# thomasfork/aircraft_trajectory_optimization

Hardware: AMD Instinct MI355X
Metric: SQP iters/sec (batched) + lap-time err vs CasADi, 50×4 collocation (higher is better)
Workload: dtype f64; 1 GPU; racetrack_parametric_esp_drone_colloc_N50_K4_cold_start_batched_sqp; N=50, K=4, nz=13, nu=4, batch_per_gpu=512, global_batch=512, max_iter=47, layout=interleaved, parallelism=instances sharded x1

## Files before the change

### aircraft_trajectory_optimization_amd/csrc/ato_capi.hip

```cpp
#include <hip/hip_runtime.h>
#include <string>
#include <exception>
#include <new>
#include <cstdlib>
#include <cstring>
#include <algorithm>
#include "ato_kernels.hpp"

#include "ato_handle.hpp"

static thread_local std::string g_last_error;

static int fail(int code, const std::string& msg) {
    g_last_error = msg;
    return code;
}

void ato_internal_set_error(const std::string& msg) { g_last_error = msg; }

#define ATO_HIP(call)                                                                        \
    do {                                                                                     \
        hipError_t e_ = (call);                                                              \
        if (e_ != hipSuccess) return fail(ATO_ERR_HIP, std::string(#call) + ": " + hipGetErrorString(e_)); \
    } while (0)
// ... 254 lines not shown
        (void)hipFree(h->d_dJ);
        h->d_dJ = nullptr;
        return fail(ATO_ERR_HIP, "hessian scratch: out of device memory");
    }
    h->hess_reserved = max_batch;
    h->hess_colors = g;
    return ATO_OK;
}

int ato_reserve(ato_handle* h, int32_t max_batch) {
    if (!h || max_batch < 1) return fail(ATO_ERR_ARG, "bad reserve arguments");
    if (h->hess_ready) {
        int rc = hess_reserve(h, max_batch);
        if (rc) return rc;
    }
    if (max_batch <= h->reserved) return ATO_OK;
    if (h->d_fpart) {
        ATO_HIP(hipDeviceSynchronize());
        ATO_HIP(hipFree(h->d_fpart));
    }
    h->d_fpart = nullptr;
    h->reserved = 0;
    ATO_HIP(hipMalloc(&h->d_fpart, (size_t)h->L.p.N * max_batch * sizeof(double)));
    h->reserved = max_batch;
    return ATO_OK;
}

}

template <class T>
static int eval_impl(ato_handle* h, int32_t batch, int32_t layout, const T* w, T* g, T* jac, T* f,
                     T* grad_f, void* stream) {
    if (!h) return fail(ATO_ERR_ARG, "null handle");
    if (batch < 1) return fail(ATO_ERR_ARG, "batch must be >= 1");
    if (layout != ATO_LAYOUT_INTERLEAVED && layout != ATO_LAYOUT_INSTANCE_MAJOR)
        return fail(ATO_ERR_ARG, "unknown layout");
    if (!w) return fail(ATO_ERR_ARG, "w is null");
    const bool wf = f || grad_f;
    if (wf && !(f && grad_f)) return fail(ATO_ERR_ARG, "f and grad_f must be requested together");
    if (wf && batch > h->reserved) {
        int rc = ato_reserve(h, batch);
        if (rc) return rc;
    }
    const bool tiled = batch > h->lf_max_batch && h->eval_tile > 0;
    const ato::ProbD& p = batch <= h->lf_max_batch || (tiled && h->tile_lf) ? h->pd_lf : h->pd;
    hipError_t e = hipSuccess;
    ato::with_model(p, [&]<class M>() {
        hipEvent_t* ev = nullptr;
        const bool sample = h->timing_stride <= 1 || h->timing_seen % h->timing_stride == 0;
        if (!h->events.empty()) ++h->timing_seen;
        if (sample && (size_t)(h->timed_calls + 1) * 3 <= h->events.size())
            ev = &h->events[(size_t)h->timed_calls++ * 3];
        e = ato::launch_eval<M, T>(p, batch, layout, w, g, jac, grad_f, f, (T*)h->d_fpart, (hipStream_t)stream,
                                   ev, tiled ? h->eval_tile : 0);
    });
    if (e != hipSuccess) return fail(ATO_ERR_HIP, std::string("kernel launch: ") + hipGetErrorString(e));
// ... 342 lines not shown
```

### aircraft_trajectory_optimization_amd/csrc/ato_ipm.hip

```cpp
#include <hip/hip_runtime.h>
#include <cmath>
#include <string>
#include "../../include/ato_ipm.h"
#include "../../include/ato.h"

void ato_internal_set_error(const std::string& msg);

namespace {

constexpr int CH = 32;
constexpr int CB = 64;
constexpr int QMAX = 9;

__device__ __forceinline__ double nmax(double a, double b) {
    return (a != a || b != b) ? __builtin_nan("") : (a > b ? a : b);
}
__device__ __forceinline__ double nmin(double a, double b) {
    return (a != a || b != b) ? __builtin_nan("") : (a < b ? a : b);
}
__device__ __forceinline__ bool fin(double v) { return fabs(v) < INFINITY; }

struct Parts {
    int len[4];
    int c0[5];
// ... 1174 lines not shown
    const int k0 = blockIdx.y * RROWS, k1 = min(n0 + m, k0 + RROWS);
    for (int k = k0 + (threadIdx.x >> 6); k < k1; k += 4) {
        const long long o = (long long)k * W + b;
        if (k < n0) {
            x[o] = xb[o];
        } else {
            const long long d = (long long)(k - n0) * W + b;
            const double y = xb[o], rp = x[o], rn = x[o + (long long)m * W];
            x[o] = (rp + y) / dp[d];
            x[o + (long long)m * W] = (rn - y) / dn[d];
            x[o + 2LL * m * W] = y;
        }
    }
}

}

extern "C" {

int ato_ipm_perturb(int32_t op, int32_t W, int32_t m, const double* prm, int64_t* hdeg, int64_t* jdeg,
                    int64_t* diters, int64_t* test, double* dx, double* dc, double* dx_last, double* dc_last,
                    const double* mu, uint8_t* pend, const int32_t* inertia, double* dw_out, double* dc_out,
                    uint8_t* tosolve, const uint8_t* fin, void* stream) {
    if (op < 0 || op > 2 || W < 0 || !prm) return fail(ATO_ERR_ARG, "ato_ipm_perturb: arguments");
    if (W == 0) return 0;
    if (!hdeg || !jdeg || !diters || !test || !dx || !dc || !dx_last || !dc_last || !mu || !pend ||
        (op == 1 && (!inertia || !dw_out || !dc_out || !tosolve)) || (op == 2 && (!tosolve || !fin)))
        return fail(ATO_ERR_ARG, "ato_ipm_perturb: arguments");
    const PertPrm o{prm[0], prm[1], prm[2], prm[3], prm[4], prm[5], prm[6], prm[7], (long long)prm[8]};
    hipLaunchKernelGGL(k_perturb, dim3((W + CB - 1) / CB), dim3(CB), 0, static_cast<hipStream_t>(stream), (int)op, W,
// ... 307 lines not shown
                       static_cast<hipStream_t>(stream), n0, m, W, x, dp, dn, xb);
    return check_launch("ato_ipm_resto_kkt_rhs");
}

int ato_ipm_resto_kkt_expand(int32_t n0, int32_t m, int32_t W, const double* xb, const double* dp, const double* dn,
                             const uint8_t* mask, double* x, void* stream) {
    if (n0 < 0 || m < 0 || W < 0 || ((n0 + m) && W && (!x || !xb || !mask || (m && (!dp || !dn)))))
        return fail(ATO_ERR_ARG, "ato_ipm_resto_kkt_expand: arguments");
    if (n0 + m == 0 || W == 0) return 0;
    if ((n0 + m + RROWS - 1) / RROWS > GRID_Y_MAX) return fail(ATO_ERR_ARG, "ato_ipm_resto_kkt_expand: too many rows");
    hipLaunchKernelGGL(k_resto_kkt_expand, dim3((W + 63) / 64, (n0 + m + RROWS - 1) / RROWS), dim3(256), 0,
                       static_cast<hipStream_t>(stream), n0, m, W, xb, dp, dn, mask, x);
    return check_launch("ato_ipm_resto_kkt_expand");
}

}
```

### aircraft_trajectory_optimization_amd/native.py

```python
import ctypes
import os
from typing import Optional, Tuple

import numpy as np

KMAX = 9
GEOM_WIDTH = 16

ATO_MODEL_DRONE, ATO_MODEL_POINT = 0, 1
ATO_ATT_ESP, ATO_ATT_YPR, ATO_ATT_DCM = 0, 1, 2
ATO_FRAME_GLOBAL, ATO_FRAME_PARAMETRIC = 0, 1
ATO_TRANS_COLLOCATION, ATO_TRANS_RK4 = 0, 1
ATO_GATE_CIRCLE, ATO_GATE_SQUARE = 0, 1
ATO_LAYOUT_INTERLEAVED, ATO_LAYOUT_INSTANCE_MAJOR = 0, 1
ATO_AUDIT_NCH = 14
ATO_GATECHECK_NCH = 9
GATE_MAX = 64
ATO_OK, ATO_ERR_ARG, ATO_ERR_UNSUPPORTED, ATO_ERR_HIP, ATO_ERR_STATE = 0, -1, -2, -3, -4
ABI_VERSION = 3
CPC_MAX = 16

_c_double_p = ctypes.POINTER(ctypes.c_double)


# ... 98 lines not shown

class AtoIpmDims(ctypes.Structure):
    _fields_ = [('n', ctypes.c_int32), ('m', ctypes.c_int32), ('mi', ctypes.c_int32), ('meq', ctypes.c_int32),
                ('iin', ctypes.c_void_p), ('ieq', ctypes.c_void_p), ('W', ctypes.c_int32)]


class AtoIpmBounds(ctypes.Structure):
    _fields_ = [('xL', ctypes.c_void_p), ('xU', ctypes.c_void_p), ('dL', ctypes.c_void_p), ('dU', ctypes.c_void_p)]


IPM_SYMBOLS = ('ato_ipm_work_size', 'ato_ipm_errors', 'ato_ipm_rhs', 'ato_ipm_direction', 'ato_ipm_measures',
               'ato_ipm_multipliers', 'ato_ipm_filter_accept', 'ato_ipm_kkt_diag', 'ato_ipm_perturb',
               'ato_ipm_status', 'ato_ipm_barrier', 'ato_ipm_filter_multi', 'ato_ipm_refine_work',
               'ato_ipm_refine_pass', 'ato_ipm_refine_decide', 'ato_ipm_resto_rows', 'ato_ipm_js_jty',
               'ato_ipm_kmul_residual', 'ato_ipm_resto_eval', 'ato_ipm_resto_hess', 'ato_ipm_resto_kkt_pack',
               'ato_ipm_resto_kkt_diag', 'ato_ipm_resto_kkt_rhs', 'ato_ipm_resto_kkt_expand')

EXPORTED_SYMBOLS = ('ato_create', 'ato_destroy', 'ato_sizes', 'ato_sparsity', 'ato_bounds',
                    'ato_reserve', 'ato_eval', 'ato_eval_f32', 'ato_hess_sparsity', 'ato_hess_eval',
                    'ato_mesh_create', 'ato_mesh_destroy', 'ato_mesh_signed_distance',
                    'ato_timing', 'ato_timing_read', 'ato_timing_stride', 'ato_last_error', 'ato_version',
                    'ato_kkt_create', 'ato_kkt_destroy', 'ato_kkt_reserve', 'ato_kkt_factor', 'ato_kkt_solve',
                    'ato_kkt_residual', 'ato_kkt_residual_list', 'ato_set_instance_spheres',
                    'ato_sphere_rows', 'ato_gradf_mode', 'ato_gradf_sparsity', 'ato_replay_set_lift',
                    'ato_replay', 'ato_remesh', 'ato_mesh_signed_distance_strided', 'ato_clearance_set_line',
                    'ato_clearance', 'ato_audit', 'ato_gatecheck', 'ato_gatecheck_set_gates',
                    'ato_gatecheck_launches') + IPM_SYMBOLS


def library_path() -> str:
    return os.environ.get('ATO_LIB_PATH') or os.path.join(os.path.dirname(os.path.abspath(__file__)), '_lib',
                                                          'libato.so')


def declare(lib: ctypes.CDLL, prefix: str = 'ato') -> ctypes.CDLL:
    vp = ctypes.c_void_p
    i32p = ctypes.POINTER(ctypes.c_int32)
    getattr(lib, f'{prefix}_last_error').restype = ctypes.c_char_p
    if prefix == 'ato':
        lib.ato_version.restype = ctypes.c_char_p
        lib.ato_create.argtypes = [ctypes.POINTER(AtoProblemDesc), ctypes.POINTER(vp)]
        lib.ato_destroy.argtypes = [vp]
        lib.ato_sizes.argtypes = [vp, i32p, i32p, i32p]
        lib.ato_sparsity.argtypes = [vp, ctypes.POINTER(i32p), ctypes.POINTER(i32p)]
        lib.ato_bounds.argtypes = [vp, _c_double_p, _c_double_p]
        lib.ato_reserve.argtypes = [vp, ctypes.c_int32]
        lib.ato_eval.argtypes = [vp, ctypes.c_int32, ctypes.c_int32, vp, vp, vp, vp, vp, vp]
        lib.ato_eval_f32.argtypes = [vp, ctypes.c_int32, ctypes.c_int32, vp, vp, vp, vp, vp, vp]
        lib.ato_hess_sparsity.argtypes = [vp, i32p, ctypes.POINTER(i32p), ctypes.POINTER(i32p), i32p]
        lib.ato_hess_eval.argtypes = [vp, ctypes.c_int32, ctypes.c_int32, vp, vp, vp, vp, vp]
        lib.ato_mesh_create.argtypes = [vp, ctypes.c_int32, vp, ctypes.c_int32, ctypes.POINTER(vp)]
        lib.ato_mesh_destroy.argtypes = [vp]
        lib.ato_mesh_signed_distance.argtypes = [vp, ctypes.c_int32, vp, vp, vp, vp]
        lib.ato_timing.argtypes = [vp, ctypes.c_int32]
        lib.ato_timing_read.argtypes = [vp, _c_double_p, _c_double_p, i32p]
        lib.ato_timing_stride.argtypes = [vp, ctypes.c_int32]
        lib.ato_set_instance_spheres.argtypes = [vp, vp, ctypes.c_int64]
        lib.ato_sphere_rows.argtypes = [vp, i32p]
        lib.ato_gradf_mode.argtypes = [vp, ctypes.c_int32]
        lib.ato_gradf_sparsity.argtypes = [vp, i32p, i32p]
        lib.ato_replay_set_lift.argtypes = [vp, vp]
# ... 34 lines not shown
        lib.ato_ipm_perturb.argtypes = [ctypes.c_int32] * 3 + [vp] * 16 + [vp]
        lib.ato_ipm_status.argtypes = [ctypes.c_int32] + [vp] * 11 + [vp]
        lib.ato_ipm_barrier.argtypes = [ctypes.c_int32] + [vp] * 10 + [vp]
        lib.ato_ipm_refine_work.argtypes = [ctypes.c_int32, ctypes.c_int32]
        lib.ato_ipm_refine_pass.argtypes = [ctypes.c_int32, ctypes.c_int32] + [vp] * 7 + [vp]
        lib.ato_ipm_refine_decide.argtypes = [ctypes.c_int32] * 4 + [vp] * 12 + [vp]
        lib.ato_ipm_resto_rows.argtypes = [ctypes.c_int32, ctypes.c_int32] + [vp] * 5 + [vp]
        lib.ato_ipm_js_jty.argtypes = [ctypes.c_int32] * 3 + [vp] * 8 + [vp]
        lib.ato_ipm_kmul_residual.argtypes = [ctypes.c_int32] * 5 + [vp] * 15 + [vp]
        lib.ato_ipm_resto_eval.argtypes = [ctypes.c_int32] * 5 + [vp] * 10 + [d] + [vp] * 3 + [vp]
        lib.ato_ipm_resto_hess.argtypes = [ctypes.c_int32] * 2 + [vp] * 7 + [vp]
        lib.ato_ipm_resto_kkt_pack.argtypes = [ctypes.c_int32] * 4 + [vp] * 9 + [vp]
        lib.ato_ipm_resto_kkt_diag.argtypes = [ctypes.c_int32] * 3 + [vp] * 9 + [vp]
        lib.ato_ipm_resto_kkt_rhs.argtypes = [ctypes.c_int32] * 3 + [vp] * 4 + [vp]
        lib.ato_ipm_resto_kkt_expand.argtypes = [ctypes.c_int32] * 3 + [vp] * 5 + [vp]
        for fn in IPM_SYMBOLS[1:]:
            getattr(lib, fn).restype = ctypes.c_int
        for fn in ('ato_create', 'ato_destroy', 'ato_sizes', 'ato_sparsity', 'ato_bounds', 'ato_reserve',
                   'ato_eval', 'ato_eval_f32', 'ato_hess_sparsity', 'ato_hess_eval', 'ato_timing',
                   'ato_timing_read', 'ato_timing_stride', 'ato_mesh_create', 'ato_mesh_destroy', 'ato_mesh_signed_distance',
                   'ato_set_instance_spheres', 'ato_sphere_rows', 'ato_gradf_mode', 'ato_gradf_sparsity',
                   'ato_replay_set_lift', 'ato_replay', 'ato_remesh', 'ato_mesh_signed_distance_strided',
                   'ato_clearance_set_line', 'ato_clearance', 'ato_audit', 'ato_gatecheck',
                   'ato_gatecheck_set_gates', 'ato_gatecheck_launches'):
            getattr(lib, fn).restype = ctypes.c_int
    return lib


_LIB: Optional[ctypes.CDLL] = None

# ... 144 lines not shown

    def gradf_nnz(self) -> int:
        return int(len(self.gradf_sparsity()))

    def set_instance_spheres(self, centres: int, stride: int):
        self._check(self.lib.ato_set_instance_spheres(self.handle, centres or None, int(stride)))

    def sphere_rows(self, P: int) -> np.ndarray:
        rows = np.zeros(P, np.int32)
        self._check(self.lib.ato_sphere_rows(self.handle, rows.ctypes.data_as(ctypes.POINTER(ctypes.c_int32))))
        return rows

    def reserve(self, max_batch: int):
        self._check(self.lib.ato_reserve(self.handle, int(max_batch)))

    def eval_ptrs(self, batch: int, w: int, g: int = 0, jac: int = 0, f: int = 0, grad_f: int = 0,
                  layout: int = ATO_LAYOUT_INTERLEAVED, stream: int = 0, fp32: bool = False):
        fn = self.lib.ato_eval_f32 if fp32 else self.lib.ato_eval
        self._check(fn(self.handle, int(batch), int(layout), w or None, g or None, jac or None,
                       f or None, grad_f or None, stream or None))

    def hess_sparsity(self) -> Tuple[np.ndarray, np.ndarray, int]:
        nnz, nc = ctypes.c_int32(), ctypes.c_int32()
        rp = ctypes.POINTER(ctypes.c_int32)()
        cp = ctypes.POINTER(ctypes.c_int32)()
        self._check(self.lib.ato_hess_sparsity(self.handle, ctypes.byref(nnz), ctypes.byref(rp), ctypes.byref(cp),
                                               ctypes.byref(nc)))
        row_ptr = np.ctypeslib.as_array(rp, shape=(self.nw + 1,)).copy()
        col = np.ctypeslib.as_array(cp, shape=(nnz.value,)).copy() if nnz.value else np.zeros(0, np.int32)
        return row_ptr, col, nc.value
# ... 100 lines not shown
```

### aircraft_trajectory_optimization_amd/solver/batched_ipm.py

```python
import os
import time
from dataclasses import dataclass, field
from typing import Dict, List, Optional

import numpy as np
import torch

from aircraft_trajectory_optimization_amd.solver.ipm import DEG_NO, DEG_UNKNOWN, DEG_YES, INF, IPMOptions, \
    T_C0X0, T_C0XP, T_CPX0, T_CPXP, T_NONE

RUNNING, OPTIMAL, ACCEPTABLE, MAX_ITER, LS_FAILED, KKT_FAILED, STOPPED, INACTIVE, TINY_STEP = range(9)
STATUS_NAMES = {RUNNING: 'running', OPTIMAL: 'optimal', ACCEPTABLE: 'acceptable', MAX_ITER: 'max_iter',
                LS_FAILED: 'restoration_failed', KKT_FAILED: 'kkt_failure', STOPPED: 'stopped',
                INACTIVE: 'inactive', TINY_STEP: 'tiny_step'}
WD_VECS = ('x', 's', 'y', 'zl', 'zu', 'vl', 'vu', 'dx', 'ds', 'dy', 'dzl', 'dzu', 'dvl', 'dvu')
WD_SCAL = ('alpha_max', 'alpha_z', 'theta', 'phi', 'gphi_d')
CSTAT = ('watchdog_started', 'watchdog_reverted', 'soft_resto_steps', 'resto_iterations', 'kkt_failures')
FILTER_MAX = 256


@dataclass
class BatchedIPMResult:
    x: torch.Tensor
    f: torch.Tensor
# ... 9 lines not shown


class BatchedDeviceEvaluator:

    def __init__(self, spec, batch: int, device: Optional[torch.device] = None, jac32: bool = False):
        from aircraft_trajectory_optimization_amd.raceline.batched import BatchedNLP
        from aircraft_trajectory_optimization_amd.raceline.evaluator import variable_stages
        self.spec = spec
        self.jac32 = bool(jac32)
        self.bn = BatchedNLP(spec, batch, device=device, buffers=False)
        self.device = self.bn.device
        self.batch = batch
        self.n, self.m, self.nnz = self.bn.sizes
        self.j_row_ptr, self.j_col = self.bn.row_ptr, self.bn.col
        self.h_row_ptr, self.h_col, _ = self.bn.problem.hess_sparsity()
        self.lbg, self.ubg = self.bn.lbg, self.bn.ubg
        self.var_stage = variable_stages(spec)
        self.counts = {'eval': 0, 'hess': 0}
        self._events: Optional[list] = None

    def timing_on(self):
        self._events = []

    def timing_total_s(self) -> float:
        if not self._events:
            return 0.0
        self._events[-1][1].synchronize()
        return sum(a.elapsed_time(b) for a, b in self._events) / 1e3

    def _tic(self):
# ... 45 lines not shown
        return ev


def _eval_into(problem, binder, B, X, n, m, nnz, jac, jac32=False):
    X = X.contiguous()
    dev = X.device
    f = torch.empty(B, dtype=torch.float64, device=dev)
    g = torch.empty((m, B), dtype=torch.float64, device=dev)
    sparse = not jac
    if getattr(problem, '_gf_sparse', None) != sparse:
        problem.gradf_mode(sparse)
        problem._gf_sparse = sparse
    if jac:
        gf = torch.empty((n, B), dtype=torch.float64, device=dev)
    else:
        scratch = binder.__dict__.setdefault('_gf_scratch', {})
        gf = scratch.get((B, dev))
        if gf is None:
            gf = scratch[(B, dev)] = torch.zeros((n, B), dtype=torch.float64, device=dev)
    J = torch.empty((nnz, B), dtype=torch.float64, device=dev) if jac and not jac32 else None
    st = torch.cuda.current_stream(dev)
    binder._bind_spheres()
    problem.eval_ptrs(B, X.data_ptr(), g=g.data_ptr(), jac=J.data_ptr() if J is not None else 0, f=f.data_ptr(),
                      grad_f=gf.data_ptr(), stream=st.cuda_stream)
    if jac and jac32:
        X32 = X.float()
        J32 = torch.empty((nnz, B), dtype=torch.float32, device=dev)
        G32 = torch.empty((m, B), dtype=torch.float32, device=dev)
        problem.eval_ptrs(B, X32.data_ptr(), g=G32.data_ptr(), jac=J32.data_ptr(), stream=st.cuda_stream, fp32=True)
        J = J32.double()
    return f, g, gf, J


def _hess_into(problem, binder, B, X, lam, sigma, nnz_h):
# ... 791 lines not shown
        nf = torch.zeros(B, dtype=torch.long, device=dev)
        n_acc = torch.zeros(B, dtype=torch.long, device=dev)
        status = torch.where(act, torch.full((B,), RUNNING, dtype=torch.long, device=dev),
                             torch.full((B,), INACTIVE, dtype=torch.long, device=dev))
        n_resto = torch.zeros(B, dtype=torch.long, device=dev)
        pert = BatchedPerturbation(o, B, dev)
        self.pert = pert
        ws_short = torch.zeros(B, dtype=torch.long, device=dev)
        in_wd = torch.zeros(B, dtype=torch.bool, device=dev)
        wd_trial = torch.zeros(B, dtype=torch.long, device=dev)
        tiny_flag = torch.zeros(B, dtype=torch.bool, device=dev)
        in_soft = torch.zeros(B, dtype=torch.bool, device=dev)
        soft_count = torch.zeros(B, dtype=torch.long, device=dev)
        wd = {}
        wd_on = o.watchdog_shortened_iter_trigger > 0
        fr_n = torch.zeros(B, dtype=torch.long, device=dev)
        fr_cnt = torch.zeros(B, dtype=torch.long, device=dev)
        fr_last = torch.zeros(B, dtype=torch.bool, device=dev)
        last_mu = torch.full((B,), -1.0, dtype=torch.float64, device=dev)
        has_acc = torch.zeros(B, dtype=torch.bool, device=dev)
        accp = {}
        cst = torch.zeros((len(CSTAT), B), dtype=torch.long, device=dev)
        wdst = torch.zeros(7, dtype=torch.long, device=dev)
        own = torch.zeros(B, dtype=torch.long, device=dev)
        waiting = torch.zeros(B, dtype=torch.bool, device=dev)
        iters = torch.zeros(B, dtype=torch.long, device=dev)
        history = []

        def add_filter(mask, th, ph):
            nonlocal F, nf
# ... 110 lines not shown
                n_acc = torch.where(act & acc_, n_acc + 1, torch.zeros_like(n_acc))
                accd = act & (n_acc >= o.acceptable_iter)
                status = torch.where(accd, torch.full_like(status, ACCEPTABLE), status)
                act = act & ~accd
                mx = act & (own >= self.lim)
                status = torch.where(mx, torch.full_like(status, MAX_ITER), status)
                act = act & ~mx
            cur_acc = act & (E0 <= o.acceptable_tol) & (du / sf <= o.acceptable_dual_inf_tol) & \
                (pr_uns <= o.acceptable_constr_viol_tol) & (co / sf <= o.acceptable_compl_inf_tol)
            n_step, n_wt, n_ac = torch.stack([act.sum(), waiting.sum(), cur_acc.sum()]).tolist()
            any_act, any_wait = n_step > 0, n_wt > 0
            if n_ac:
                cur_pt = {'x': x, 's': s, 'y': y, 'zl': zl, 'zu': zu, 'vl': vl, 'vu': vu}
                if not accp:
                    accp = {k_: torch.zeros_like(v_) for k_, v_ in cur_pt.items()}
                accp = {k_: torch.where(cur_acc[None, :], cur_pt[k_], v_) for k_, v_ in accp.items()}
                has_acc = has_acc | cur_acc
            if not any_act and not any_wait and not inflight:
                break
            self.step_counter.add(n_step, self.in_resto_phase)
            if on_iteration is not None:
                on_iteration(it, int(n_step), self.step_counter)
            laps.lap('check')
            stepping = act.clone()
            resto = torch.zeros(B, dtype=torch.bool, device=dev)
            kresto = resto
            if progress and it % progress == 0:
                import sys
                print(f'[batched ipm{" resto" if stop_check is not None else ""}] iter {it}: '
                      f'{int(act.sum())} active, {int((status == OPTIMAL).sum())} optimal', file=sys.stderr, flush=True)
            if any_act:
# ... 101 lines not shown
                soft_try = soft_now & ~soft_over
                dirs = {'dx': dx, 'ds': ds, 'dy': dy, 'dzl': dzl, 'dzu': dzu, 'dvl': dvl, 'dvu': dvu}
                nosoc = torch.zeros_like(act)
                wdm = torch.zeros_like(act)
                any_kwd = any_wd = False
                if wd_on:
                    start = act & ~tiny & ~in_wd & ~kwd & ~in_soft & (ws_short >= o.watchdog_shortened_iter_trigger)
                    wdm = act & ~kwd & (in_wd | start)
                    any_start, any_kwd, any_wd = torch.stack([start.any(), kwd.any(), wdm.any()]).tolist()
                    if any_start:
                        cur = {'x': x, 's': s, 'y': y, 'zl': zl, 'zu': zu, 'vl': vl, 'vu': vu, **dirs,
                               'alpha_max': alpha_max, 'alpha_z': alpha_z, 'theta': theta, 'phi': phi,
                               'gphi_d': gphi_d}
                        if not wd:
                            wd = {k: torch.zeros_like(cur[k]) for k in WD_VECS + WD_SCAL}
                        wd = {k: torch.where(start[None, :] if v.dim() == 2 else start, cur[k], v)
                              for k, v in wd.items()}
                        in_wd = in_wd | start
                        wd_trial = torch.where(start, torch.zeros_like(wd_trial), wd_trial)
                        wdst[0] += start.sum()
                        cst[0] += start.long()

                def revert(msk):
                    nonlocal x, s, y, zl, zu, vl, vu, alpha_max, alpha_z, theta, phi, gphi_d, in_wd, nosoc, \
                        f, g, gf, jv
                    m2 = msk[None, :]
                    x, s, y = (torch.where(m2, wd[k], v) for k, v in (('x', x), ('s', s), ('y', y)))
                    zl, zu, vl, vu = (torch.where(m2, wd[k], v) for k, v in (('zl', zl), ('zu', zu), ('vl', vl),
                                                                           ('vu', vu)))
                    for k in dirs:
                        dirs[k] = torch.where(m2, wd[k], dirs[k])
                    alpha_max, alpha_z, theta, phi, gphi_d = (
                        torch.where(msk, wd[k], v) for k, v in (('alpha_max', alpha_max), ('alpha_z', alpha_z),
                                                                ('theta', theta), ('phi', phi), ('gphi_d', gphi_d)))
                    in_wd = in_wd & ~msk
                    nosoc = nosoc | msk
                    fe_, ge_, gfe_, jve_ = self._eval(x)
                    f, g = torch.where(msk, fe_, f), torch.where(m2, ge_, g)
                    gf, jv = torch.where(m2, gfe_, gf), torch.where(m2, jve_, jv)
                    wdst[2] += msk.sum()
                    cst[1] += msk.long()

                def alpha_min_of(theta_, gphi_):
                    neg = gphi_ < 0
                    mgd = torch.clamp(-gphi_, min=1e-300)
                    t1 = o.gamma_phi * theta_ / mgd
                    t2 = o.delta * theta_ ** o.s_theta / mgd ** o.s_phi
                    amin = torch.where(neg & (theta_ <= self.theta_min),
                                       torch.clamp(torch.minimum(t1, t2), max=o.gamma_theta),
                                       torch.where(neg, torch.clamp(t1, max=o.gamma_theta),
                                                   torch.full_like(t1, o.gamma_theta)))
                    return o.alpha_min_frac * amin

                if any_kwd:
# ... 4 lines not shown
                wd_succ = torch.zeros_like(act)
                wd_cols = wdm.clone()
                pend = act & ~soft_now
                resto = torch.zeros(B, dtype=torch.bool, device=dev)
                first = torch.ones(B, dtype=torch.bool, device=dev)
                xn, sn = x.clone(), s.clone()
                an, dyn = torch.zeros_like(alpha), dy.clone()
                armn = torch.zeros(B, dtype=torch.bool, device=dev)
                fresh = pend.clone()
                fresh_any = True
                accf = torch.zeros(B, dtype=torch.bool, device=dev)
                frs = (fr_n, fr_cnt, fr_last)

                def take(mask, al, xt, st, arm, dyt):
                    nonlocal xn, sn, an, dyn, armn, accf
                    m2 = mask[None, :]
                    xn = torch.where(m2, xt, xn)
                    sn = torch.where(m2, st, sn)
                    an = torch.where(mask, al, an)
                    dyn = torch.where(m2, dyt, dyn)
                    armn = torch.where(mask, arm, armn)
                    accf = torch.where(mask, fresh, accf)

                laps.lap('direction')
                lsfail = torch.zeros_like(act)
                for _ls in range(200):
                    failed = pend & ~(alpha > alpha_min)
                    if o.ls_first_trial:
                        failed = failed & ~fresh
                    any_failed, n_left = torch.stack([failed.any(), (pend & ~failed).sum()]).tolist()
# ... 17 lines not shown
                            0, torch.where(acc_p, kacc, K).long())
                        acc = torch.zeros_like(pend).index_copy(0, pidx, acc_p)
                        mf = torch.zeros_like(pend).index_copy(0, pidx, mfail)
                        alpha = alpha.index_copy(0, pidx, a_p)
                        take(acc, alpha, x + alpha * dx, s + alpha * ds, torch.zeros_like(pend).index_copy(0, pidx, marm),
                             dy)
                        lsfail = lsfail | mf
                        pend = pend & ~acc & ~mf
                        continue
                    xt = x + alpha * dx
                    st = s + alpha * ds
                    laps.lap('ls_logic')
                    ft, gt = self._eval_fg(xt)
                    laps.lap('ls_eval')
                    tht, pht = self._measures(xt, st, gt, ft, mu)
                    if _ls == 0 and any_wd:
                        th_r, ph_r = torch.where(wdm, wd['theta'], theta), torch.where(wdm, wd['phi'], phi)
                        gd_r, al_r = torch.where(wdm, wd['gphi_d'], gphi_d), torch.where(wdm, wd['alpha_max'], alpha)
                    else:
                        th_r, ph_r, gd_r, al_r = theta, phi, gphi_d, alpha
                    okt, armt, soc = self._filter_test(th_r, ph_r, gd_r, al_r, tht, pht, F, nf,
                                                       pend & ~tiny if _ls == 0 else pend, first, frs)
                    soc = soc & ~nosoc & ~wdm & ~tiny
                    take(okt, alpha, xt, st, armt, dy)
                    pend = pend & ~okt
                    if _ls == 0:
                        take(tiny, alpha, xt, st, torch.ones_like(tiny), dy)
                        pend = pend & ~tiny
                        if any_wd:
                            wd_succ = wdm & okt
                            in_wd = in_wd & ~wd_succ
# ... 44 lines not shown
                    wdst[6] += (soft_sat & in_soft).sum()
                    in_soft = torch.where(soft_ok, ~soft_sat, in_soft)
                    soft_count = torch.where(soft_ok & soft_sat, torch.zeros_like(soft_count),
                                             torch.where(enter & soft_ok, torch.zeros_like(soft_count), soft_count))
                failed_all = (lsfail & ~soft_ok) | soft_over | (soft_try & ~soft_ok)
                if allow_restoration:
                    resto = failed_all | kresto
                    if o.resto_feasible_fact > 0:
                        near = resto & (theta <= o.resto_feasible_fact * o.tol)
                        back = near & has_acc
                        status = torch.where(back, torch.full_like(status, ACCEPTABLE),
                                             torch.where(near, torch.full_like(status, LS_FAILED), status))
                        act = act & ~near
                        resto = resto & ~near
                        e0_stale[cols[back]] = True
                        if accp:
                            b2 = back[None, :]
                            x, s, y = (torch.where(b2, accp[k_], v_) for k_, v_ in (('x', x), ('s', s), ('y', y)))
                            zl, zu, vl, vu = (torch.where(b2, accp[k_], v_) for k_, v_ in
                                              (('zl', zl), ('zu', zu), ('vl', vl), ('vu', vu)))
                else:
                    status = torch.where(failed_all, torch.full_like(status, LS_FAILED), status)
                    act = act & ~failed_all
                    resto = kresto & False
                laps.lap('ls_logic')
                upd = act & ~resto
                if any_wd:
                    theta = torch.where(wd_succ, wd['theta'], theta)
                    phi = torch.where(wd_succ, wd['phi'], phi)
                armn = torch.where(soft_ok, ~soft_sat, armn)
                add_filter(upd & ~armn, theta, phi)
                if wd_on:
                    normal = upd & ~tiny & ~wd_cols & ~soft_ok
                    short = ~accf if o.watchdog_ipopt_counter else an < alpha_max
                    ws_short = torch.where(normal, torch.where(short, ws_short + 1, torch.zeros_like(ws_short)),
                                           torch.where(upd & ~soft_ok, torch.zeros_like(ws_short), ws_short))
                wdst[3] += tiny.sum()
                m2 = upd[None, :]
                x = torch.where(m2, xn, x)
                s = torch.where(m2, sn, s)
                fe, ge, gfe, jve = self._eval(x)
                f = torch.where(upd, fe, f)
                g = torch.where(m2, ge, g)
                gf = torch.where(m2, gfe, gf)
                jv = torch.where(m2, jve, jv)
                laps.lap('ls_eval')
                y = torch.where(m2, y + an * dyn, y)
                az = torch.where(upd, torch.where(soft_ok, al_soft, alpha_z), torch.zeros_like(alpha_z))
                zl, zu, vl, vu = kappa_sigma(zl, zu, vl, vu, az, (dzl, dzu, dvl, dvu))
            own = own + stepping.long()
            laps.lap('accept')
            waiting = waiting | resto
            act = act & ~resto
            in_soft = in_soft & ~resto
            n_act, n_wait = torch.stack([act.sum(), waiting.sum()]).tolist()
            done = None
            if inflight:
                ready = [j for j in inflight if j['future'].done()]
                if not ready and n_act == 0 and (not n_wait or len(inflight) >= self.ASYNC_PHASES):
                    import concurrent.futures as cf
                    cf.wait([j['future'] for j in inflight], return_when=cf.FIRST_COMPLETED)
                    ready = [j for j in inflight if j['future'].done()]
# ... 28 lines not shown
                        done = self._restore(can, state, theta_w, F, nf)
            if done is not None:
                can, xr, sr, okr, hitm, kr = done
                R = can
                resto_ran = True
                laps.lap('resto')
                own = own + torch.where(can, kr, torch.zeros_like(kr))
                cst[3] += torch.where(can, kr, torch.zeros_like(kr))
                bad = can & ~okr & ~hitm
                status = torch.where(bad, torch.full_like(status, LS_FAILED), status)
                status = torch.where(hitm, torch.full_like(status, MAX_ITER), status)
                moved = okr | hitm
                if bool(moved.any()):
                    r2 = moved[None, :]
                    x0_, s0_ = x, s
                    x = torch.where(r2, xr, x)
                    s = torch.where(r2, sr, s)
                    fe, ge, gfe, jve = self._eval(x)
                    f = torch.where(moved, fe, f)
                    g = torch.where(r2, ge, g)
                    gf = torch.where(r2, gfe, gf)
                    jv = torch.where(r2, jve, jv)
                    nz = self._post_resto_bound_mults(x0_, s0_, x, s, zl, zu, vl, vu, mu, tau)
                    zl, zu, vl, vu = (torch.where(r2, a_, b_) for a_, b_ in zip(nz, (zl, zu, vl, vu)))
                    ynew = torch.zeros_like(y)
                    if o.constr_mult_reset_threshold > 0:
                        ynew = self._ls_multipliers(jv * sg[self.jr], gf, zl, zu, vl, vu, okr,
                                                    ymax=o.constr_mult_reset_threshold)
                    y = torch.where(r2, ynew, y)
                    zc = kappa_sigma(zl, zu, vl, vu, torch.zeros_like(mu), (zl, zu, vl, vu))
                    zl, zu, vl, vu = (torch.where(r2, a_, b_) for a_, b_ in zip(zc, (zl, zu, vl, vu)))
                    iters = torch.where(moved, own, iters)
                    act = act | okr
                laps.lap('resto_post')

        else:
            e0_stale[cols[stepping]] = True
        if on_iteration is not None:
            on_iteration(it, -1, self.step_counter)
        for j in inflight:
            R, xr, sr, okr, hitm, kr = self._resto_collect(j, cols, x, s, B0)
            e0_stale[cols[R]] = True
            x = torch.where(((R & okr) | hitm)[None, :], xr, x)
            s = torch.where(((R & okr) | hitm)[None, :], sr, s)
            status = torch.where((R & okr) | hitm, torch.full_like(status, MAX_ITER), status)
            status = torch.where(R & ~okr & ~hitm & (status == RUNNING), torch.full_like(status, LS_FAILED), status)
# ... 533 lines not shown
```

### aircraft_trajectory_optimization_amd/solver/ipm_device.py

```python
import ctypes
from typing import Dict, Tuple

import numpy as np
import torch

from aircraft_trajectory_optimization_amd import native


def _p(t):
    return ctypes.c_void_p(t.data_ptr()) if t is not None else None


def resto_rows(dr, dp, dn):
    m, W = dr.shape
    for t in (dr, dp, dn):
        if t.dtype != torch.float64 or t.shape != (m, W) or not t.is_cuda:
            raise ValueError('resto_rows: expected fp64 [m, W] device tensors')
    dr, dp, dn = dr.contiguous(), dp.contiguous(), dn.contiguous()
    drow = torch.empty_like(dr)
    cnt = torch.zeros((W, 2), dtype=torch.int32, device=dr.device)
    lib = native.load()
    rc = lib.ato_ipm_resto_rows(m, W, _p(dr), _p(dp), _p(dn), _p(drow), _p(cnt),
                                ctypes.c_void_p(torch.cuda.current_stream(dr.device).cuda_stream))
    if rc != 0:
# ... 185 lines not shown
def resto_kkt_expand(n0, m, xb, dp, dn, mask, x):
    W = x.shape[1]
    dev = x.device
    _own2('resto_kkt_expand x', x, n0 + 3 * m, W, dev)
    if not x.is_cuda:
        raise ValueError('resto_kkt_expand: expected device tensors')
    xb = _f64('resto_kkt_expand xb', xb, n0 + m, W, dev)
    dp, dn = _f64('resto_kkt_expand dp', dp, m, W, dev), _f64('resto_kkt_expand dn', dn, m, W, dev)
    mask = _i32('resto_kkt_expand mask', mask, W, dev, torch.bool)
    lib = native.load()
    _rc(lib, lib.ato_ipm_resto_kkt_expand(n0, m, W, _p(xb), _p(dp), _p(dn), _p(mask), _p(x), _stream_of(dev)),
        'ato_ipm_resto_kkt_expand')
    return x


class DeviceIPMKernels:
    def __init__(self, n: int, m: int, iin: torch.Tensor, ieq: torch.Tensor, device):
        self.lib = native.load()
        self.device = torch.device(device)
        self.n, self.m = int(n), int(m)
        self.iin = iin.to(device=self.device, dtype=torch.int32).contiguous()
        self.ieq = ieq.to(device=self.device, dtype=torch.int32).contiguous()
        self.mi, self.meq = len(self.iin), len(self.ieq)
        self._dims: Dict[int, native.AtoIpmDims] = {}
        self._work: Dict[int, torch.Tensor] = {}
        self._prm: Dict[tuple, np.ndarray] = {}

    def dims(self, W: int):
        d = self._dims.get(W)
        if d is None:
            d = native.AtoIpmDims(self.n, self.m, self.mi, self.meq, _p(self.iin) if self.mi else None,
# ... 275 lines not shown
```

### include/ato.h

```cpp
#ifndef ATO_H
#define ATO_H

#include <stdint.h>

#ifdef __cplusplus
extern "C" {
#endif

#define ATO_ABI_VERSION 3
#define ATO_KMAX 9
#define ATO_GEOM_WIDTH 16

enum { ATO_OK = 0, ATO_ERR_ARG = -1, ATO_ERR_UNSUPPORTED = -2, ATO_ERR_HIP = -3,
       ATO_ERR_STATE = -4 };

enum { ATO_MODEL_DRONE = 0, ATO_MODEL_POINT = 1 };
enum { ATO_ATT_ESP = 0, ATO_ATT_YPR = 1, ATO_ATT_DCM = 2 };
enum { ATO_FRAME_GLOBAL = 0, ATO_FRAME_PARAMETRIC = 1 };
enum { ATO_TRANS_COLLOCATION = 0, ATO_TRANS_RK4 = 1 };
enum { ATO_GATE_CIRCLE = 0, ATO_GATE_SQUARE = 1 };
#define ATO_CPC_MAX 16
enum { ATO_LAYOUT_INTERLEAVED = 0, ATO_LAYOUT_INSTANCE_MAJOR = 1 };

typedef struct ato_gate {
// ... 48 lines not shown

int ato_create(const ato_problem_desc* desc, ato_handle** out);
int ato_destroy(ato_handle* h);

int ato_sizes(const ato_handle* h, int32_t* nw, int32_t* ng, int32_t* nnz);

int ato_sparsity(const ato_handle* h, const int32_t** row_ptr, const int32_t** col);

int ato_bounds(const ato_handle* h, double* lbg, double* ubg);

int ato_gradf_sparsity(const ato_handle* h, int32_t* nnz, int32_t* idx);

int ato_gradf_mode(ato_handle* h, int32_t sparse);

int ato_reserve(ato_handle* h, int32_t max_batch);

int ato_eval(ato_handle* h, int32_t batch, int32_t layout, const double* w,
             double* g, double* jac, double* f, double* grad_f, void* stream);

int ato_eval_f32(ato_handle* h, int32_t batch, int32_t layout, const float* w,
                 float* g, float* jac, float* f, float* grad_f, void* stream);

int ato_hess_sparsity(ato_handle* h, int32_t* nnz, const int32_t** row_ptr, const int32_t** col,
                      int32_t* n_colors);

int ato_hess_eval(ato_handle* h, int32_t batch, int32_t layout, const double* w, const double* lam,
                  const double* sigma, double* hess, void* stream);

int ato_set_instance_spheres(ato_handle* h, const double* centres, int64_t stride);

// ... 59 lines not shown
```

### include/ato_ipm.h

```cpp
#ifndef ATO_IPM_H
#define ATO_IPM_H

#include <stddef.h>
#include <stdint.h>

#ifdef __cplusplus
extern "C" {
#endif

typedef struct ato_ipm_dims {
    int32_t n;
    int32_t m;
    int32_t mi;
    int32_t meq;
    const int32_t* iin;
    const int32_t* ieq;
    int32_t W;
} ato_ipm_dims;

typedef struct ato_ipm_bounds {
    const double* xL;
    const double* xU;
    const double* dL;
    const double* dU;
// ... 76 lines not shown
                       const double* jv, const double* sg, const double* x_ref, const double* dr2,
                       const double* zeta, double rho, double* gr, double* gfr, double* jr, void* stream);
int ato_ipm_resto_hess(int32_t nnz, int32_t W, const int32_t* src, const int32_t* dcol, const double* H0,
                       const double* sigma, const double* zeta, const double* dr2, double* h, void* stream);
int ato_ipm_resto_kkt_pack(int32_t nh, int32_t nj, int32_t n0, int32_t W, const int32_t* h_map,
                           const int32_t* pos_orig, const int32_t* h_diag, const uint8_t* diag_new, const double* H,
                           const double* J, double* Hb, double* Jb, double* hd, void* stream);
int ato_ipm_resto_kkt_diag(int32_t n0, int32_t m, int32_t W, const double* dx, const double* dr, const double* hd,
                           const uint8_t* mask, double* dxb, double* drow, double* dp, double* dn, int32_t* cnt,
                           void* stream);
int ato_ipm_resto_kkt_rhs(int32_t n0, int32_t m, int32_t W, const double* x, const double* dp, const double* dn,
                          double* xb, void* stream);
int ato_ipm_resto_kkt_expand(int32_t n0, int32_t m, int32_t W, const double* xb, const double* dp, const double* dn,
                             const uint8_t* mask, double* x, void* stream);

#ifdef __cplusplus
}
#endif
#endif
```

Baseline: 7100 SQP iterations/s (instance-iterations of the batched interior-point solve, all GPUs).

## Fuse masked column-select torch.where chains into one multi-array HIP kernel

Adds a batched select kernel that applies a per-instance column mask to up to 16 arrays (fp64/int64/bool) in a single launch, optionally in place. The IPM line search, watchdog, accept and restoration paths use it instead of many separate torch.where calls, which cuts kernel-launch and temporary-allocation overhead. It also splits eval scratch reservation from Hessian reservation, pre-reserves eval scratch for the multi-trial line search, and shares a flat grad-f scratch buffer across batch sizes. The new path is on by default behind an env flag. In-place updates change aliasing semantics compared with the old functional where calls.

```diff
diff --git a/aircraft_trajectory_optimization_amd/csrc/ato_capi.hip b/aircraft_trajectory_optimization_amd/csrc/ato_capi.hip
--- a/aircraft_trajectory_optimization_amd/csrc/ato_capi.hip
+++ b/aircraft_trajectory_optimization_amd/csrc/ato_capi.hip
@@ -292,6 +292,11 @@
         int rc = hess_reserve(h, max_batch);
         if (rc) return rc;
     }
+    return ato_eval_reserve(h, max_batch);
+}
+
+int ato_eval_reserve(ato_handle* h, int32_t max_batch) {
+    if (!h || max_batch < 1) return fail(ATO_ERR_ARG, "bad reserve arguments");
     if (max_batch <= h->reserved) return ATO_OK;
     if (h->d_fpart) {
         ATO_HIP(hipDeviceSynchronize());
@@ -317,7 +322,7 @@
     const bool wf = f || grad_f;
     if (wf && !(f && grad_f)) return fail(ATO_ERR_ARG, "f and grad_f must be requested together");
     if (wf && batch > h->reserved) {
-        int rc = ato_reserve(h, batch);
+        int rc = ato_eval_reserve(h, batch);
         if (rc) return rc;
     }
     const bool tiled = batch > h->lf_max_batch && h->eval_tile > 0;
diff --git a/aircraft_trajectory_optimization_amd/csrc/ato_ipm.hip b/aircraft_trajectory_optimization_amd/csrc/ato_ipm.hip
--- a/aircraft_trajectory_optimization_amd/csrc/ato_ipm.hip
+++ b/aircraft_trajectory_optimization_amd/csrc/ato_ipm.hip
@@ -1212,6 +1212,57 @@
     }
 }
 
+constexpr int SEL_MAX = 16;
+
+struct SelArgs {
+    const void* src[SEL_MAX];
+    const void* dst[SEL_MAX];
+    void* out[SEL_MAX];
+    int rows[SEL_MAX];
+    int b0[SEL_MAX + 1];
+    int wide[SEL_MAX];
+};
+
+template <class T>
+__device__ __forceinline__ void select_rows(int W, int b, int r0, int r1, bool m, const void* src, const void* dst,
+                                            void* out) {
+    const T* s = static_cast<const T*>(src);
+    const T* d = static_cast<const T*>(dst);
+    T* o = static_cast<T*>(out);
+    for (int r = r0 + (threadIdx.x >> 6); r < r1; r += 4) {
+        const long long i = (long long)r * W + b;
+        o[i] = m ? s[i] : d[i];
+    }
+}
+
+__global__ __launch_bounds__(256) void k_select_cols(int W, int count, SelArgs a, const uint8_t* __restrict__ mask) {
+    const int b = blockIdx.x * 64 + (threadIdx.x & 63);
+    if (b >= W) return;
+    const int y = blockIdx.y;
+    const void* src = a.src[0];
+    const void* dst = a.dst[0];
+    void* out = a.out[0];
+    int rows = a.rows[0], first = a.b0[0], wide = a.wide[0];
+#pragma unroll
+    for (int k = 1; k < SEL_MAX; ++k) {
+        if (k < count && y >= a.b0[k]) {
+            src = a.src[k];
+            dst = a.dst[k];
+            out = a.out[k];
+            rows = a.rows[k];
+            first = a.b0[k];
+            wide = a.wide[k];
+        }
+    }
+    const bool m = mask[b] != 0;
+    if (!m && out == dst) return;
+    const int r0 = (y - first) * RROWS, r1 = min(rows, r0 + RROWS);
+    if (wide)
+        select_rows<unsigned long long>(W, b, r0, r1, m, src, dst, out);
+    else
+        select_rows<uint8_t>(W, b, r0, r1, m, src, dst, out);
+}
+
 }
 
 extern "C" {
@@ -1549,4 +1600,31 @@
     return check_launch("ato_ipm_resto_kkt_expand");
 }
 
-}
+int ato_ipm_select_cols(int32_t W, int32_t count, const int32_t* rows, const int32_t* esize, const void* const* src,
+                        void* const* dst, void* const* out, const uint8_t* mask, void* stream) {
+    if (W < 0 || count < 0 || count > SEL_MAX || (count && (!rows || !esize || !src || !dst)))
+        return fail(ATO_ERR_ARG, "ato_ipm_select_cols: arguments");
+    SelArgs a{};
+    long long blocks = 0;
+    for (int k = 0; k < count; ++k) {
+        if (rows[k] < 0 || (esize[k] != 1 && esize[k] != 8))
+            return fail(ATO_ERR_ARG, "ato_ipm_select_cols: row count or element size");
+        if (rows[k] && W && (!src[k] || !dst[k] || (out && !out[k]) || !mask))
+            return fail(ATO_ERR_ARG, "ato_ipm_select_cols: null array");
+        a.src[k] = src[k];
+        a.dst[k] = dst[k];
+        a.out[k] = out ? out[k] : dst[k];
+        a.rows[k] = rows[k];
+        a.wide[k] = esize[k] == 8;
+        a.b0[k] = (int)blocks;
+        blocks += ((long long)rows[k] + RROWS - 1) / RROWS;
+        if (blocks > GRID_Y_MAX) return fail(ATO_ERR_ARG, "ato_ipm_select_cols: too many rows");
+    }
+    for (int k = count; k <= SEL_MAX; ++k) a.b0[k] = (int)blocks;
+    if (W == 0 || blocks == 0) return 0;
+    hipLaunchKernelGGL(k_select_cols, dim3((W + 63) / 64, (unsigned)blocks), dim3(256), 0,
+                       static_cast<hipStream_t>(stream), W, count, a, mask);
+    return check_launch("ato_ipm_select_cols");
+}
+
+}
diff --git a/aircraft_trajectory_optimization_amd/native.py b/aircraft_trajectory_optimization_amd/native.py
--- a/aircraft_trajectory_optimization_amd/native.py
+++ b/aircraft_trajectory_optimization_amd/native.py
@@ -136,7 +136,7 @@
                'ato_ipm_status', 'ato_ipm_barrier', 'ato_ipm_filter_multi', 'ato_ipm_refine_work',
                'ato_ipm_refine_pass', 'ato_ipm_refine_decide', 'ato_ipm_resto_rows', 'ato_ipm_js_jty',
                'ato_ipm_kmul_residual', 'ato_ipm_resto_eval', 'ato_ipm_resto_hess', 'ato_ipm_resto_kkt_pack',
-               'ato_ipm_resto_kkt_diag', 'ato_ipm_resto_kkt_rhs', 'ato_ipm_resto_kkt_expand')
+               'ato_ipm_resto_kkt_diag', 'ato_ipm_resto_kkt_rhs', 'ato_ipm_resto_kkt_expand', 'ato_ipm_select_cols')
 
 EXPORTED_SYMBOLS = ('ato_create', 'ato_destroy', 'ato_sizes', 'ato_sparsity', 'ato_bounds',
                     'ato_reserve', 'ato_eval', 'ato_eval_f32', 'ato_hess_sparsity', 'ato_hess_eval',
@@ -147,7 +147,7 @@
                     'ato_sphere_rows', 'ato_gradf_mode', 'ato_gradf_sparsity', 'ato_replay_set_lift',
                     'ato_replay', 'ato_remesh', 'ato_mesh_signed_distance_strided', 'ato_clearance_set_line',
                     'ato_clearance', 'ato_audit', 'ato_gatecheck', 'ato_gatecheck_set_gates',
-                    'ato_gatecheck_launches') + IPM_SYMBOLS
+                    'ato_gatecheck_launches', 'ato_eval_reserve') + IPM_SYMBOLS
 
 
 def library_path() -> str:
@@ -167,6 +167,8 @@
         lib.ato_sparsity.argtypes = [vp, ctypes.POINTER(i32p), ctypes.POINTER(i32p)]
         lib.ato_bounds.argtypes = [vp, _c_double_p, _c_double_p]
         lib.ato_reserve.argtypes = [vp, ctypes.c_int32]
+        lib.ato_eval_reserve.argtypes = [vp, ctypes.c_int32]
+        lib.ato_eval_reserve.restype = ctypes.c_int
         lib.ato_eval.argtypes = [vp, ctypes.c_int32, ctypes.c_int32, vp, vp, vp, vp, vp, vp]
         lib.ato_eval_f32.argtypes = [vp, ctypes.c_int32, ctypes.c_int32, vp, vp, vp, vp, vp, vp]
         lib.ato_hess_sparsity.argtypes = [vp, i32p, ctypes.POINTER(i32p), ctypes.POINTER(i32p), i32p]
@@ -231,6 +233,7 @@
         lib.ato_ipm_resto_kkt_diag.argtypes = [ctypes.c_int32] * 3 + [vp] * 9 + [vp]
         lib.ato_ipm_resto_kkt_rhs.argtypes = [ctypes.c_int32] * 3 + [vp] * 4 + [vp]
         lib.ato_ipm_resto_kkt_expand.argtypes = [ctypes.c_int32] * 3 + [vp] * 5 + [vp]
+        lib.ato_ipm_select_cols.argtypes = [ctypes.c_int32] * 2 + [vp] * 6 + [vp]
         for fn in IPM_SYMBOLS[1:]:
             getattr(lib, fn).restype = ctypes.c_int
         for fn in ('ato_create', 'ato_destroy', 'ato_sizes', 'ato_sparsity', 'ato_bounds', 'ato_reserve',
@@ -405,6 +408,9 @@
     def reserve(self, max_batch: int):
         self._check(self.lib.ato_reserve(self.handle, int(max_batch)))
 
+    def eval_reserve(self, max_batch: int):
+        self._check(self.lib.ato_eval_reserve(self.handle, int(max_batch)))
+
     def eval_ptrs(self, batch: int, w: int, g: int = 0, jac: int = 0, f: int = 0, grad_f: int = 0,
                   layout: int = ATO_LAYOUT_INTERLEAVED, stream: int = 0, fp32: bool = False):
         fn = self.lib.ato_eval_f32 if fp32 else self.lib.ato_eval
diff --git a/aircraft_trajectory_optimization_amd/solver/batched_ipm.py b/aircraft_trajectory_optimization_amd/solver/batched_ipm.py
--- a/aircraft_trajectory_optimization_amd/solver/batched_ipm.py
+++ b/aircraft_trajectory_optimization_amd/solver/batched_ipm.py
@@ -47,6 +47,7 @@
         self.n, self.m, self.nnz = self.bn.sizes
         self.j_row_ptr, self.j_col = self.bn.row_ptr, self.bn.col
         self.h_row_ptr, self.h_col, _ = self.bn.problem.hess_sparsity()
+        self.bn.problem.eval_reserve(max(1, BatchedInteriorPoint.LS_MULTI_K) * batch)
         self.lbg, self.ubg = self.bn.lbg, self.bn.ubg
         self.var_stage = variable_stages(spec)
         self.counts = {'eval': 0, 'hess': 0}
@@ -122,10 +123,12 @@
     if jac:
         gf = torch.empty((n, B), dtype=torch.float64, device=dev)
     else:
-        scratch = binder.__dict__.setdefault('_gf_scratch', {})
-        gf = scratch.get((B, dev))
-        if gf is None:
-            gf = scratch[(B, dev)] = torch.zeros((n, B), dtype=torch.float64, device=dev)
+        root = getattr(binder, 'base', binder)
+        scratch = root.__dict__.setdefault('_gf_scratch', {})
+        flat = scratch.get(dev)
+        if flat is None or flat.numel() < n * B:
+            flat = scratch[dev] = torch.zeros(n * B, dtype=torch.float64, device=dev)
+        gf = flat[:n * B].view(n, B)
     J = torch.empty((nnz, B), dtype=torch.float64, device=dev) if jac and not jac32 else None
     st = torch.cuda.current_stream(dev)
     binder._bind_spheres()
@@ -947,6 +950,8 @@
         soft_count = torch.zeros(B, dtype=torch.long, device=dev)
         wd = {}
         wd_on = o.watchdog_shortened_iter_trigger > 0
+        fused = self.vk is not None and os.environ.get('ATO_IPM_FUSED_STEP', '1') != '0'
+        merge_cols = self.vk.select_cols if fused else None
         fr_n = torch.zeros(B, dtype=torch.long, device=dev)
         fr_cnt = torch.zeros(B, dtype=torch.long, device=dev)
         fr_last = torch.zeros(B, dtype=torch.bool, device=dev)
@@ -1087,7 +1092,10 @@
                 cur_pt = {'x': x, 's': s, 'y': y, 'zl': zl, 'zu': zu, 'vl': vl, 'vu': vu}
                 if not accp:
                     accp = {k_: torch.zeros_like(v_) for k_, v_ in cur_pt.items()}
-                accp = {k_: torch.where(cur_acc[None, :], cur_pt[k_], v_) for k_, v_ in accp.items()}
+                if fused:
+                    merge_cols(cur_acc, [cur_pt[k_] for k_ in accp], list(accp.values()), inplace=True)
+                else:
+                    accp = {k_: torch.where(cur_acc[None, :], cur_pt[k_], v_) for k_, v_ in accp.items()}
                 has_acc = has_acc | cur_acc
             if not any_act and not any_wait and not inflight:
                 break
@@ -1219,8 +1227,11 @@
                                'gphi_d': gphi_d}
                         if not wd:
                             wd = {k: torch.zeros_like(cur[k]) for k in WD_VECS + WD_SCAL}
-                        wd = {k: torch.where(start[None, :] if v.dim() == 2 else start, cur[k], v)
-                              for k, v in wd.items()}
+                        if fused:
+                            merge_cols(start, [cur[k] for k in wd], list(wd.values()), inplace=True)
+                        else:
+                            wd = {k: torch.where(start[None, :] if v.dim() == 2 else start, cur[k], v)
+                                  for k, v in wd.items()}
                         in_wd = in_wd | start
                         wd_trial = torch.where(start, torch.zeros_like(wd_trial), wd_trial)
                         wdst[0] += start.sum()
@@ -1230,19 +1241,33 @@
                     nonlocal x, s, y, zl, zu, vl, vu, alpha_max, alpha_z, theta, phi, gphi_d, in_wd, nosoc, \
                         f, g, gf, jv
                     m2 = msk[None, :]
-                    x, s, y = (torch.where(m2, wd[k], v) for k, v in (('x', x), ('s', s), ('y', y)))
-                    zl, zu, vl, vu = (torch.where(m2, wd[k], v) for k, v in (('zl', zl), ('zu', zu), ('vl', vl),
-                                                                           ('vu', vu)))
-                    for k in dirs:
-                        dirs[k] = torch.where(m2, wd[k], dirs[k])
-                    alpha_max, alpha_z, theta, phi, gphi_d = (
-                        torch.where(msk, wd[k], v) for k, v in (('alpha_max', alpha_max), ('alpha_z', alpha_z),
-                                                                ('theta', theta), ('phi', phi), ('gphi_d', gphi_d)))
+                    if fused:
+                        pt = ('x', 's', 'y', 'zl', 'zu', 'vl', 'vu')
+                        sc = ('alpha_max', 'alpha_z', 'theta', 'phi', 'gphi_d')
+                        new = merge_cols(msk, [wd[k] for k in pt + tuple(dirs) + sc],
+                                         [x, s, y, zl, zu, vl, vu, *dirs.values(), alpha_max, alpha_z, theta, phi,
+                                          gphi_d])
+                        x, s, y, zl, zu, vl, vu = new[:7]
+                        for k, v in zip(tuple(dirs), new[7:7 + len(dirs)]):
+                            dirs[k] = v
+                        alpha_max, alpha_z, theta, phi, gphi_d = new[7 + len(dirs):]
+                    else:
+                        x, s, y = (torch.where(m2, wd[k], v) for k, v in (('x', x), ('s', s), ('y', y)))
+                        zl, zu, vl, vu = (torch.where(m2, wd[k], v) for k, v in (('zl', zl), ('zu', zu), ('vl', vl),
+                                                                               ('vu', vu)))
+                        for k in dirs:
+                            dirs[k] = torch.where(m2, wd[k], dirs[k])
+                        alpha_max, alpha_z, theta, phi, gphi_d = (
+                            torch.where(msk, wd[k], v) for k, v in (('alpha_max', alpha_max), ('alpha_z', alpha_z),
+                                                                    ('theta', theta), ('phi', phi), ('gphi_d', gphi_d)))
                     in_wd = in_wd & ~msk
                     nosoc = nosoc | msk
                     fe_, ge_, gfe_, jve_ = self._eval(x)
-                    f, g = torch.where(msk, fe_, f), torch.where(m2, ge_, g)
-                    gf, jv = torch.where(m2, gfe_, gf), torch.where(m2, jve_, jv)
+                    if fused:
+                        f, g, gf, jv = merge_cols(msk, [fe_, ge_, gfe_, jve_], [f, g, gf, jv])
+                    else:
+                        f, g = torch.where(msk, fe_, f), torch.where(m2, ge_, g)
+                        gf, jv = torch.where(m2, gfe_, gf), torch.where(m2, jve_, jv)
                     wdst[2] += msk.sum()
                     cst[1] += msk.long()
 
@@ -1277,6 +1302,9 @@
 
                 def take(mask, al, xt, st, arm, dyt):
                     nonlocal xn, sn, an, dyn, armn, accf
+                    if fused:
+                        merge_cols(mask, [xt, st, al, dyt, arm, fresh], [xn, sn, an, dyn, armn, accf], inplace=True)
+                        return
                     m2 = mask[None, :]
                     xn = torch.where(m2, xt, xn)
                     sn = torch.where(m2, st, sn)
@@ -1324,7 +1352,10 @@
                     ft, gt = self._eval_fg(xt)
                     laps.lap('ls_eval')
                     tht, pht = self._measures(xt, st, gt, ft, mu)
-                    if _ls == 0 and any_wd:
+                    if _ls == 0 and any_wd and fused:
+                        th_r, ph_r, gd_r, al_r = merge_cols(
+                            wdm, [wd['theta'], wd['phi'], wd['gphi_d'], wd['alpha_max']], [theta, phi, gphi_d, alpha])
+                    elif _ls == 0 and any_wd:
                         th_r, ph_r = torch.where(wdm, wd['theta'], theta), torch.where(wdm, wd['phi'], phi)
                         gd_r, al_r = torch.where(wdm, wd['gphi_d'], gphi_d), torch.where(wdm, wd['alpha_max'], alpha)
                     else:
@@ -1399,7 +1430,11 @@
                         act = act & ~near
                         resto = resto & ~near
                         e0_stale[cols[back]] = True
-                        if accp:
+                        if accp and fused:
+                            x, s, y, zl, zu, vl, vu = merge_cols(
+                                back, [accp[k_] for k_ in ('x', 's', 'y', 'zl', 'zu', 'vl', 'vu')],
+                                [x, s, y, zl, zu, vl, vu])
+                        elif accp:
                             b2 = back[None, :]
                             x, s, y = (torch.where(b2, accp[k_], v_) for k_, v_ in (('x', x), ('s', s), ('y', y)))
                             zl, zu, vl, vu = (torch.where(b2, accp[k_], v_) for k_, v_ in
@@ -1422,15 +1457,21 @@
                                            torch.where(upd & ~soft_ok, torch.zeros_like(ws_short), ws_short))
                 wdst[3] += tiny.sum()
                 m2 = upd[None, :]
-                x = torch.where(m2, xn, x)
-                s = torch.where(m2, sn, s)
-                fe, ge, gfe, jve = self._eval(x)
-                f = torch.where(upd, fe, f)
-                g = torch.where(m2, ge, g)
-                gf = torch.where(m2, gfe, gf)
-                jv = torch.where(m2, jve, jv)
-                laps.lap('ls_eval')
-                y = torch.where(m2, y + an * dyn, y)
+                if fused:
+                    x, s = merge_cols(upd, [xn, sn], [x, s])
+                    fe, ge, gfe, jve = self._eval(x)
+                    f, g, gf, jv, y = merge_cols(upd, [fe, ge, gfe, jve, y + an * dyn], [f, g, gf, jv, y])
+                    laps.lap('ls_eval')
+                else:
+                    x = torch.where(m2, xn, x)
+                    s = torch.where(m2, sn, s)
+                    fe, ge, gfe, jve = self._eval(x)
+                    f = torch.where(upd, fe, f)
+                    g = torch.where(m2, ge, g)
+                    gf = torch.where(m2, gfe, gf)
+                    jv = torch.where(m2, jve, jv)
+                    laps.lap('ls_eval')
+                    y = torch.where(m2, y + an * dyn, y)
                 az = torch.where(upd, torch.where(soft_ok, al_soft, alpha_z), torch.zeros_like(alpha_z))
                 zl, zu, vl, vu = kappa_sigma(zl, zu, vl, vu, az, (dzl, dzu, dvl, dvu))
             own = own + stepping.long()
@@ -1489,22 +1530,34 @@
                 if bool(moved.any()):
                     r2 = moved[None, :]
                     x0_, s0_ = x, s
-                    x = torch.where(r2, xr, x)
-                    s = torch.where(r2, sr, s)
-                    fe, ge, gfe, jve = self._eval(x)
-                    f = torch.where(moved, fe, f)
-                    g = torch.where(r2, ge, g)
-                    gf = torch.where(r2, gfe, gf)
-                    jv = torch.where(r2, jve, jv)
+                    if fused:
+                        x, s = merge_cols(moved, [xr, sr], [x, s])
+                        fe, ge, gfe, jve = self._eval(x)
+                        f, g, gf, jv = merge_cols(moved, [fe, ge, gfe, jve], [f, g, gf, jv])
+                    else:
+                        x = torch.where(r2, xr, x)
+                        s = torch.where(r2, sr, s)
+                        fe, ge, gfe, jve = self._eval(x)
+                        f = torch.where(moved, fe, f)
+                        g = torch.where(r2, ge, g)
+                        gf = torch.where(r2, gfe, gf)
+                        jv = torch.where(r2, jve, jv)
                     nz = self._post_resto_bound_mults(x0_, s0_, x, s, zl, zu, vl, vu, mu, tau)
-                    zl, zu, vl, vu = (torch.where(r2, a_, b_) for a_, b_ in zip(nz, (zl, zu, vl, vu)))
+                    if fused:
+                        zl, zu, vl, vu = merge_cols(moved, nz, [zl, zu, vl, vu])
+                    else:
+                        zl, zu, vl, vu = (torch.where(r2, a_, b_) for a_, b_ in zip(nz, (zl, zu, vl, vu)))
                     ynew = torch.zeros_like(y)
                     if o.constr_mult_reset_threshold > 0:
                         ynew = self._ls_multipliers(jv * sg[self.jr], gf, zl, zu, vl, vu, okr,
                                                     ymax=o.constr_mult_reset_threshold)
-                    y = torch.where(r2, ynew, y)
-                    zc = kappa_sigma(zl, zu, vl, vu, torch.zeros_like(mu), (zl, zu, vl, vu))
-                    zl, zu, vl, vu = (torch.where(r2, a_, b_) for a_, b_ in zip(zc, (zl, zu, vl, vu)))
+                    if fused:
+                        zc = kappa_sigma(zl, zu, vl, vu, torch.zeros_like(mu), (zl, zu, vl, vu))
+                        y, zl, zu, vl, vu = merge_cols(moved, [ynew, *zc], [y, zl, zu, vl, vu])
+                    else:
+                        y = torch.where(r2, ynew, y)
+                        zc = kappa_sigma(zl, zu, vl, vu, torch.zeros_like(mu), (zl, zu, vl, vu))
+                        zl, zu, vl, vu = (torch.where(r2, a_, b_) for a_, b_ in zip(zc, (zl, zu, vl, vu)))
                     iters = torch.where(moved, own, iters)
                     act = act | okr
                 laps.lap('resto_post')
diff --git a/aircraft_trajectory_optimization_amd/solver/ipm_device.py b/aircraft_trajectory_optimization_amd/solver/ipm_device.py
--- a/aircraft_trajectory_optimization_amd/solver/ipm_device.py
+++ b/aircraft_trajectory_optimization_amd/solver/ipm_device.py
@@ -223,7 +223,54 @@
     return x
 
 
+SELECT_MAX = 16
+_SELECT_ESIZE = {torch.float64: 8, torch.int64: 8, torch.bool: 1}
+
+
+def select_cols(mask, src, dst, inplace=False):
+    src, dst = list(src), list(dst)
+    if len(src) != len(dst):
+        raise ValueError('select_cols: as many sources as destinations')
+    if not dst:
+        return []
+    W = mask.shape[0]
+    dev = mask.device
+    if mask.dtype != torch.bool or mask.dim() != 1 or not mask.is_cuda:
+        raise ValueError('select_cols: expected a bool [W] device mask')
+    mask = mask.contiguous()
+    outs, keep = [], []
+    for k, (s, d) in enumerate(zip(src, dst)):
+        if d.dtype not in _SELECT_ESIZE or d.dim() not in (1, 2) or d.shape[-1] != W or d.device != dev:
+            raise ValueError(f'select_cols: array {k}: expected fp64 / int64 / bool [rows, {W}] or [{W}] on {dev}, '
+                             f'got {tuple(d.shape)} {d.dtype} {d.device}')
+        if s.dtype != d.dtype or s.shape != d.shape or s.device != dev:
+            raise ValueError(f'select_cols: array {k}: source {tuple(s.shape)} {s.dtype} {s.device} does not match '
+                             f'its destination {tuple(d.shape)} {d.dtype}')
+        if inplace:
+            if not d.is_contiguous():
+                raise ValueError(f'select_cols: array {k}: an array updated in place must be contiguous')
+            outs.append(d)
+        else:
+            d = d.contiguous()
+            outs.append(torch.empty_like(d, memory_format=torch.contiguous_format))
+        keep.append((s.contiguous(), d))
+    lib = native.load()
+    st = _stream_of(dev)
+    for k0 in range(0, len(outs), SELECT_MAX):
+        part = range(k0, min(k0 + SELECT_MAX, len(outs)))
+        cnt = len(part)
+        rows = (ctypes.c_int32 * cnt)(*[outs[k].numel() // W if W else 0 for k in part])
+        esz = (ctypes.c_int32 * cnt)(*[_SELECT_ESIZE[outs[k].dtype] for k in part])
+        ps = (ctypes.c_void_p * cnt)(*[keep[k][0].data_ptr() or None for k in part])
+        pd = (ctypes.c_void_p * cnt)(*[keep[k][1].data_ptr() or None for k in part])
+        po = None if inplace else (ctypes.c_void_p * cnt)(*[outs[k].data_ptr() or None for k in part])
+        _rc(lib, lib.ato_ipm_select_cols(W, cnt, rows, esz, ps, pd, po, _p(mask), st), 'ato_ipm_select_cols')
+    return outs
+
+
 class DeviceIPMKernels:
+    select_cols = staticmethod(select_cols)
+
     def __init__(self, n: int, m: int, iin: torch.Tensor, ieq: torch.Tensor, device):
         self.lib = native.load()
         self.device = torch.device(device)
diff --git a/include/ato.h b/include/ato.h
--- a/include/ato.h
+++ b/include/ato.h
@@ -86,6 +86,7 @@
 int ato_gradf_mode(ato_handle* h, int32_t sparse);
 
 int ato_reserve(ato_handle* h, int32_t max_batch);
+int ato_eval_reserve(ato_handle* h, int32_t max_batch);
 
 int ato_eval(ato_handle* h, int32_t batch, int32_t layout, const double* w,
              double* g, double* jac, double* f, double* grad_f, void* stream);
diff --git a/include/ato_ipm.h b/include/ato_ipm.h
--- a/include/ato_ipm.h
+++ b/include/ato_ipm.h
@@ -114,6 +114,9 @@
 int ato_ipm_resto_kkt_expand(int32_t n0, int32_t m, int32_t W, const double* xb, const double* dp, const double* dn,
                              const uint8_t* mask, double* x, void* stream);
 
+int ato_ipm_select_cols(int32_t W, int32_t count, const int32_t* rows, const int32_t* esize, const void* const* src,
+                        void* const* dst, void* const* out, const uint8_t* mask, void* stream);
+
 #ifdef __cplusplus
 }
 #endif
```

Measured after the change: 6963 SQP iterations/s (instance-iterations of the batched interior-point solve, all GPUs). -1.9%, worse.
